# jackra1n/raytracer-rust

Hardware: NVIDIA B200
Metric: Mpaths/s (semesterbild 800x600x256spp, depth 30) (higher is better)
Workload: dtype f32

## Files before the change

raytracer-rust_b200/csrc/pt_bvh8.h:

```cpp
#pragma once
#include "pt_math.h"
#include "pt_types.h"

namespace pt {

struct MeshHit {
  float t;
  uint32_t tri;
  uint32_t order;
};

PT_HD float box_rcp(float x) {
#if defined(__CUDA_ARCH__)
  float r;
  asm("rcp.approx.ftz.f32 %0, %1;" : "=f"(r) : "f"(x));
  return r;
#else
  return 1.0f / x;
#endif
}

template <int J>
PT_HD float byte_as_unit_float(uint32_t packed) {
#if defined(__CUDA_ARCH__)
// ... 22 lines not shown
  uint32_t octinv;
  uint2 ng;
  uint2 tg;
  uint2 tg2;
};

PT_HD void trav_begin(TravState &s, V3 o, V3 d, float t_min, float t_max) {
  s.o = o;
  s.d = d;
  s.idx = box_rcp(d.x), s.idy = box_rcp(d.y), s.idz = box_rcp(d.z);
  s.t_min = t_min;
  s.best_t = t_max;
  s.best_order = 0u;
  s.best_tri = 0xffffffffu;
  const uint32_t sx = f2u(d.x) >> 31, sy = f2u(d.y) >> 31, sz = f2u(d.z) >> 31;
  s.octinv = 7u - (sx | (sy << 1) | (sz << 2));
  s.ng = make_uint2(0u, 0x80000000u);
  s.tg = make_uint2(0u, 0u);
  s.tg2 = make_uint2(0u, 0u);
}
PT_HD bool trav_has_node(const TravState &s) { return s.ng.y > 0x00FFFFFFu; }
PT_HD bool trav_has_tri(const TravState &s) { return s.tg.y != 0u; }

template <bool COUNT>
PT_HD void trav_node(const DMesh &m, TravState &s, uint2 *stack, int &sp, TraversalCounters *ctr) {
  const uint32_t hits = s.ng.y, imask = hits & 0xffu;
  const int bit = 31 - clz32(hits);
  s.ng.y &= ~(1u << bit);
  if (s.ng.y > 0x00FFFFFFu) stack[sp++] = s.ng;
  const uint32_t slot = (uint32_t)(bit - 24) ^ s.octinv;
  const uint32_t rel = (uint32_t)popc32(imask & ~(0xFFFFFFFFu << slot));
  const float4 *np = m.nodes + (size_t)(s.ng.x + rel) * 5;
  const float4 q0 = ldg4(np), q1 = ldg4(np + 1), q2 = ldg4(np + 2), q3 = ldg4(np + 3), q4 = ldg4(np + 4);
  if (COUNT) ctr->nodes++;

  const uint32_t e = f2u(q0.w);
  const float adjx = u2f(((e & 0xffu) + 15u) << 23) * s.idx;
  const float adjy = u2f((((e >> 8) & 0xffu) + 15u) << 23) * s.idy;
  const float adjz = u2f((((e >> 16) & 0xffu) + 15u) << 23) * s.idz;
  const float orgx = (q0.x - s.o.x) * s.idx - adjx, orgy = (q0.y - s.o.y) * s.idy - adjy, orgz = (q0.z - s.o.z) * s.idz - adjz;

  const bool sx = (f2u(s.d.x) >> 31) != 0u, sy = (f2u(s.d.y) >> 31) != 0u, sz = (f2u(s.d.z) >> 31) != 0u;
  const uint32_t lox0 = f2u(q2.x), lox1 = f2u(q2.y), loy0 = f2u(q2.z), loy1 = f2u(q2.w);
  const uint32_t loz0 = f2u(q3.x), loz1 = f2u(q3.y), hix0 = f2u(q3.z), hix1 = f2u(q3.w);
  const uint32_t hiy0 = f2u(q4.x), hiy1 = f2u(q4.y), hiz0 = f2u(q4.z), hiz1 = f2u(q4.w);
  const uint32_t nx[2] = {sx ? hix0 : lox0, sx ? hix1 : lox1}, fx[2] = {sx ? lox0 : hix0, sx ? lox1 : hix1};
  const uint32_t ny[2] = {sy ? hiy0 : loy0, sy ? hiy1 : loy1}, fy[2] = {sy ? loy0 : hiy0, sy ? loy1 : hiy1};
  const uint32_t nz[2] = {sz ? hiz0 : loz0, sz ? hiz1 : loz1}, fz[2] = {sz ? loz0 : hiz0, sz ? loz1 : hiz1};
  const uint32_t meta[2] = {f2u(q1.z), f2u(q1.w)};
  const uint32_t octinv4 = s.octinv * 0x01010101u;

  uint32_t hitmask = 0u;
#pragma unroll
  for (int h = 0; h < 2; h++) {
    const uint32_t meta4 = meta[h];
    const uint32_t is_inner4 = (meta4 & (meta4 << 1)) & 0x10101010u;
    const uint32_t inner_mask4 = (is_inner4 >> 4) * 0xffu;
    const uint32_t bit_index4 = (meta4 ^ (octinv4 & inner_mask4)) & 0x1f1f1f1fu;
    const uint32_t child_bits4 = (meta4 >> 5) & 0x07070707u;
#define PT_CHILD2(J)                                                                                                  \
  {                                                                                                                   \
    float tnx0, tnx1, tny0, tny1, tnz0, tnz1, tfx0, tfx1, tfy0, tfy1, tfz0, tfz1;                                     \
    fma2_bcast(tnx0, tnx1, byte_as_unit_float<J>(nx[h]), byte_as_unit_float<J + 1>(nx[h]), adjx, orgx);               \
    fma2_bcast(tny0, tny1, byte_as_unit_float<J>(ny[h]), byte_as_unit_float<J + 1>(ny[h]), adjy, orgy);               \
    fma2_bcast(tnz0, tnz1, byte_as_unit_float<J>(nz[h]), byte_as_unit_float<J + 1>(nz[h]), adjz, orgz);               \
    fma2_bcast(tfx0, tfx1, byte_as_unit_float<J>(fx[h]), byte_as_unit_float<J + 1>(fx[h]), adjx, orgx);               \
    fma2_bcast(tfy0, tfy1, byte_as_unit_float<J>(fy[h]), byte_as_unit_float<J + 1>(fy[h]), adjy, orgy);               \
    fma2_bcast(tfz0, tfz1, byte_as_unit_float<J>(fz[h]), byte_as_unit_float<J + 1>(fz[h]), adjz, orgz);               \
             \
    const float tn0 = fmaxf(fmaxf(tnx0, tny0), fmaxf(tnz0, s.t_min)), tf0 = fminf(fminf(tfx0, tfy0), fminf(tfz0, s.best_t)); \
    const float tn1 = fmaxf(fmaxf(tnx1, tny1), fmaxf(tnz1, s.t_min)), tf1 = fminf(fminf(tfx1, tfy1), fminf(tfz1, s.best_t)); \
    if (tn0 <= tf0) hitmask |= ((child_bits4 >> (8 * (J))) & 0xffu) << ((bit_index4 >> (8 * (J))) & 0xffu);           \
    if (tn1 <= tf1) hitmask |= ((child_bits4 >> (8 * (J + 1))) & 0xffu) << ((bit_index4 >> (8 * (J + 1))) & 0xffu);   \
  }
    PT_CHILD2(0) PT_CHILD2(2)
#undef PT_CHILD
  }
  s.ng.x = f2u(q1.x);
  s.ng.y = (hitmask & 0xFF000000u) | (e >> 24);
  const uint2 leaf_hits = make_uint2(f2u(q1.y), hitmask & 0x00FFFFFFu);
  if (s.tg.y == 0u) s.tg = leaf_hits;
  else s.tg2 = leaf_hits;
}

template <bool COUNT>
PT_HD void trav_tri(const DMesh &m, TravState &s, TraversalCounters *ctr) {
  const int bit = 31 - clz32(s.tg.y);
  const float4 *tp = m.tris + (size_t)(s.tg.x + (uint32_t)bit) * 3;
  s.tg.y &= ~(1u << bit);
  if (s.tg.y == 0u) {
    s.tg = s.tg2;
    s.tg2 = make_uint2(0u, 0u);
  }
  const float4 t0 = ldg4(tp), t1 = ldg4(tp + 1), t2 = ldg4(tp + 2);
  if (COUNT) ctr->tris++;
  const V3 v0 = v3(t0.x, t0.y, t0.z), edge1 = v3(t1.x, t1.y, t1.z), edge2 = v3(t2.x, t2.y, t2.z);
  const V3 h = cross(s.d, edge2);
  const float a = dot(edge1, h);
  if (fabsf(a) < kEps) return;
  const float f = 1.0f / a;
  const V3 sv = s.o - v0;
  const float u = f * dot(sv, h);
  if (!(0.0f <= u && u <= 1.0f)) return;
  const V3 q = cross(sv, edge1);
  const float v = f * dot(s.d, q);
  if (v < 0.0f || u + v > 1.0f) return;
  const float t = f * dot(edge2, q);
  if (!(t > s.t_min)) return;
  const uint32_t order = f2u(t1.w);
  if (t < s.best_t || (t == s.best_t && order < s.best_order)) {
    s.best_t = t;
    s.best_order = order;
    s.best_tri = f2u(t0.w);
  }
}

template <bool COUNT>
PT_HD bool bvh8_closest(const DMesh &m, V3 o, V3 d, float t_min, float t_max, MeshHit &out, TraversalCounters *ctr) {
  TravState s;
  trav_begin(s, o, d, t_min, t_max);
  uint2 stack[kTraversalStack];
  int sp = 0;
  for (;;) {
    if (trav_has_tri(s)) {
      trav_tri<COUNT>(m, s, ctr);
    } else if (trav_has_node(s)) {
      trav_node<COUNT>(m, s, stack, sp, ctr);
    } else {
      if (sp == 0) break;
      s.ng = stack[--sp];
    }
  }
  if (s.best_tri == 0xffffffffu) return false;
  out.t = s.best_t;
  out.tri = s.best_tri;
  out.order = s.best_order;
  return true;
}

}
```

raytracer-rust_b200/csrc/pt_scene_host.h:

```cpp
#pragma once
#include <algorithm>
#include <cmath>
#include <cstring>
#include <memory>
#include <stdexcept>
#include <vector>

#include "../../include/ptcore.h"
#include "pt_build.h"
#include "pt_types.h"

namespace pt {

inline DMesh make_dmesh(const MeshBuild &m, const float4 *nodes, const float4 *tris, const float4 *normals) {
  DMesh d;
  d.nodes = nodes;
  d.tris = tris;
  d.normals = normals;
  d.n_nodes = (int32_t)m.nodes.size();
  d.n_tris = (int32_t)m.tri48.size();
  for (int a = 0; a < 3; a++) d.root_lo[a] = m.root_lo[a], d.root_hi[a] = m.root_hi[a];
  return d;
}

struct HostScene {
  std::vector<DMaterial> materials;
  std::vector<DObject> objects;
  std::vector<std::unique_ptr<MeshBuild>> meshes;
  std::vector<float> sky;
  int32_t sky_w = 0, sky_h = 0;
  std::vector<DLight> lights;
  std::vector<float> sky_dist;

  int add_material(const ptc_material *m) {
    if (m->type < PTC_MAT_LAMBERT || m->type > PTC_MAT_NULL) throw std::invalid_argument("unknown material type");
    DMaterial d;
    memset(&d, 0, sizeof(d));
    d.type = m->type;
    d.distribution = m->distribution;
    d.fuzz = m->fuzz;
    d.ior = m->ior;
    d.roughness = m->roughness;
    d.inv_scale = m->inv_scale;
    for (int i = 0; i < 3; i++) {
// ... 146 lines not shown
```

raytracer-rust_b200/csrc/pt_types.h:

```cpp
#pragma once
#include "pt_hd.h"

namespace pt {

enum ObjType : int32_t { OBJ_SPHERE = 0, OBJ_PLANE = 1, OBJ_QUAD = 2, OBJ_CUBE = 3, OBJ_MESH = 4 };

struct alignas(16) DObject {
  int32_t type;
  int32_t material;
  int32_t mesh;
  int32_t hit_bits;
  float f[32];
};
static_assert(sizeof(DObject) == 144, "DObject layout");

struct alignas(16) DMaterial {
  int32_t type;
  int32_t distribution;
  float fuzz, ior;
  float albedo[3];
  float roughness;
  float off_color[3];
  float inv_scale;
  float eta[3];
  float pad0;
  float k[3];
  float pad1;
};
static_assert(sizeof(DMaterial) == 80, "DMaterial layout");

struct alignas(16) Node8 {
  float4 q[5];
};
static_assert(sizeof(Node8) == 80, "Node8 layout");

struct alignas(16) Tri48 {
  float4 t[3];
};

struct DMesh {
  const float4 *nodes;
  const float4 *tris;
  const float4 *normals;
  int32_t n_nodes, n_tris;
  float root_lo[3], root_hi[3];
};

struct alignas(16) DLight {
  int32_t type;
  int32_t object;
  float area;
  float pad;
  float f[12];
  float emission[3];
  float pad2;
};
constexpr int kMaxLights = 63;

struct SkyDist {
  const float *marg, *cos, *inv_sa, *cond;
  int32_t wc, hc;
};
PT_HD int32_t sky_cells(int32_t texels) { return texels > 1 ? texels - 1 : 1; }
PT_HD size_t sky_dist_size(int32_t w, int32_t h) {
  const size_t wc = (size_t)sky_cells(w), hc = (size_t)sky_cells(h);
  return 3 * hc + 2 + hc * (wc + 1);
}
PT_HD SkyDist sky_dist_view(const float *p, int32_t w, int32_t h) {
// ... 40 lines not shown
```

raytracer-rust_b200/csrc/pt_wavefront.cuh:

```cuda
#pragma once
#include <cuda_runtime.h>

#include "../../include/ptcore.h"
#include "pt_bsdf.h"
#include "pt_philox.h"
#include "pt_prims.h"

namespace ptw {
using namespace pt;

constexpr int kBlock = 256;
constexpr int kSegPerSM = 4;
constexpr uint32_t kRefillLanes = 8;
constexpr uint32_t kNoSteal = 0x80000000u;
constexpr unsigned long long kNoTriHit = ~0ull;

struct Ctl {
  unsigned long long next_path;
  unsigned long long total_paths;
  unsigned long long rays;
  unsigned long long nodes, tris, mesh_rays;
  uint32_t n_active;
  uint32_t sync_timeouts;
  uint32_t iterations[2];
// ... 101 lines not shown
      if (!mesh_root_may_hit(sc.meshes[ob->mesh], mr, t_min, closest)) continue;
      park_ray = mr;
      return k;
    }
    if (type == OBJ_SPHERE) hit = hit_sphere(ob->f, ray, t_min, closest, best);
    else if (type == OBJ_QUAD) hit = hit_quad(ob->f, ray, t_min, closest, best);
    else if (type == OBJ_CUBE) hit = hit_cube_t(ob->f, ray, t_min, closest, best);
    else hit = hit_plane(ob->f, ray, t_min, closest, best);
    if (hit) {
      improved = true;
      closest = best.t;
      best.object = k;
      best.triangle = -1;
      best.material = ob->hit_bits;
    }
  }
  return -1;
}

__device__ __forceinline__ void finish_hit(const DObject *objs, const Ray &ray, Hit &best) {
  if (best.front_face == kCubeNormalPending) cube_finish_normal(objs[best.object].f, ray, best);
}

constexpr int kSmemObjects = 24;
template <bool kSharedObjs>
__device__ __forceinline__ const DObject *stage_objects(const DScene &sc, DObject *s_objs) {
  if (!kSharedObjs) return sc.objects;
  const uint4 *src = reinterpret_cast<const uint4 *>(sc.objects);
  uint4 *dst = reinterpret_cast<uint4 *>(s_objs);
  const int n16 = sc.n_objects * (int)(sizeof(DObject) / 16);
  for (int i = threadIdx.x; i < n16; i += blockDim.x) dst[i] = src[i];
  return s_objs;
}

__device__ __forceinline__ void park_tasks(uint32_t *s_ntask, const TaskQ &tq, int par, uint32_t seg_base, int park, uint32_t i,
                                           const MeshRay &mr, float closest) {
  const uint32_t lane = threadIdx.x & 31u;
  const uint32_t mask = __ballot_sync(0xffffffffu, park >= 0);
  if (mask == 0u) return;
  uint32_t slot0 = 0;
  if (lane == 0) slot0 = atomicAdd(s_ntask, (uint32_t)__popc(mask));
  slot0 = __shfl_sync(0xffffffffu, slot0, 0);
  if (park >= 0) {
    const uint32_t slot = seg_base + slot0 + (uint32_t)__popc(mask & ((1u << lane) - 1u));
    tq.ray[par][slot] = make_uint2(i, (uint32_t)park);
    tq.o[par][slot] = make_float4(mr.o.x, mr.o.y, mr.o.z, closest);
    tq.d[par][slot] = make_float4(mr.d.x, mr.d.y, mr.d.z, 0.0f);
    tq.res[par][slot] = kNoTriHit;
  }
}

template <bool kSharedObjs>
__device__ __forceinline__ void stage_pre(uint32_t seg, uint32_t n_seg, const DScene &sc, const ExtendOut &out, const TaskQ &tq,
                                          float t_min, float t_max) {
  __shared__ uint32_t s_ntask;
  __shared__ __align__(16) DObject s_objs[kSmemObjects];
  const uint32_t tid = threadIdx.x;
  const uint32_t n = out.b.cnt[seg], seg_base = seg * out.b.cap;
  if (tid == 0) s_ntask = 0;
  const DObject *objs = kSharedObjs ? s_objs : sc.objects;
  stage_objects<kSharedObjs>(sc, s_objs);
  __syncthreads();
  for (uint32_t c0 = 0; c0 < n; c0 += (uint32_t)kBlock) {
    const uint32_t i = seg_base + c0 + tid;
    int park = -1;
    MeshRay mr;
    float closest = t_max;
    if (c0 + tid < n) {
      const float4 o4 = out.b.ray_o[i], d4 = out.b.ray_d[i];
      const Ray ray{v3(o4.x, o4.y, o4.z), v3(d4.x, d4.y, d4.z)};
      Hit best;
      bool improved = false;
      park = scan_objects(sc, objs, ray, t_min, closest, best, improved, 0, mr);
      if (improved) finish_hit(objs, ray, best);
      if (improved) write_hit(out, i, best);
      else write_miss(out, i);
    }
    park_tasks(&s_ntask, tq, 0, seg_base, park, i, mr, closest);
  }
  __syncthreads();
  if (tid == 0 && tq.cnt) tq.cnt[seg] = s_ntask;
  (void)n_seg;
}

template <bool COUNT>
__device__ __forceinline__ void stage_traverse(uint32_t seg, uint32_t n_seg, Ctl *ctl, const DScene &sc, const TaskQ &tq, int round,
                                               float t_min, uint32_t cap, uint32_t refill_arg, uint32_t part = 0u, uint32_t parts = 1u) {
  __shared__ uint32_t s_cur;
  const uint32_t n_all = tq.cnt[(uint32_t)round * n_seg + seg];
  const uint32_t first = (uint32_t)((unsigned long long)n_all * part / parts);
  const uint32_t n = (uint32_t)((unsigned long long)n_all * (part + 1u) / parts) - first, seg_base = seg * cap + first;
  const int par = round & 1;
  const uint32_t lane = threadIdx.x & 31u;
  const uint32_t lt_mask = (1u << lane) - 1u;
  const uint32_t refill_lanes = refill_arg & ~kNoSteal;
  const bool steal = (refill_arg & kNoSteal) == 0u;
  const uint32_t quota = (n >= (uint32_t)kBlock || !steal) ? 32u : max(1u, (n + (uint32_t)(kBlock / 32) - 1u) / (uint32_t)(kBlock / 32));
  if (threadIdx.x == 0) s_cur = 0;
  __syncthreads();
  TraversalCounters tc{0u, 0u, 0u};
  TravState s;
  DMesh mesh;
  mesh.nodes = nullptr, mesh.tris = nullptr;
  uint2 stack[kTraversalStack];
  int sp = 0, sb = 0;
  bool active = false;
  uint32_t task = 0;
  bool exhausted = n == 0u;
  s.ng = make_uint2(0u, 0u);
  for (;;) {
    const uint32_t idle = __ballot_sync(0xffffffffu, !active);
    if (!exhausted && (idle == 0xffffffffu || (uint32_t)__popc(idle) >= refill_lanes)) {
      const uint32_t cnt = min((uint32_t)__popc(idle), quota);
      uint32_t base = 0;
      if (lane == 0) base = atomicAdd(&s_cur, cnt);
      base = __shfl_sync(0xffffffffu, base, 0);
      const uint32_t my_rank = (uint32_t)__popc(idle & lt_mask);
      if (!active && my_rank < cnt) {
        const uint32_t j = base + my_rank;
        if (j < n) {
          const uint32_t slot = seg_base + j;
          const uint2 rk = tq.ray[par][slot];
          const float4 o4 = tq.o[par][slot], d4 = __ldcs(&tq.d[par][slot]);
          const DMesh *gm = sc.meshes + sc.objects[rk.y].mesh;
          mesh.nodes = gm->nodes;
          mesh.tris = gm->tris;
          trav_begin(s, v3(o4.x, o4.y, o4.z), v3(d4.x, d4.y, d4.z), t_min, o4.w);
          sp = sb = 0;
          task = slot;
          active = true;
          if (COUNT) tc.mesh_rays++;
        }
      }
      if (base + cnt >= n) exhausted = true;
    } else if (steal && exhausted && idle != 0u && idle != 0xffffffffu) {
      const bool can_give = active && (sp > sb || __popc(s.ng.y >> 24) >= 2);
      const uint32_t donors = __ballot_sync(0xffffffffu, can_give);
      if (donors != 0u) {
        const uint32_t pairs = (uint32_t)min(__popc(idle), __popc(donors));
        const bool give = can_give && (uint32_t)__popc(donors & lt_mask) < pairs;
        const uint32_t my_idle_rank = (uint32_t)__popc(idle & lt_mask);
        const bool take = !active && my_idle_rank < pairs;
        uint2 entry = make_uint2(0u, 0u);
        if (give) {
          if (sp > sb) {
            entry = stack[sb++];
          } else {
            const uint32_t pend = s.ng.y & 0xFF000000u, bit = pend & (0u - pend);
            entry = make_uint2(s.ng.x, bit | (s.ng.y & 0xffu));
            s.ng.y &= ~bit;
          }
        }
        const int src = take ? (int)__fns(donors, 0u, (int)my_idle_rank + 1) : (int)lane;
        const float ox = __shfl_sync(0xffffffffu, s.o.x, src), oy = __shfl_sync(0xffffffffu, s.o.y, src), oz = __shfl_sync(0xffffffffu, s.o.z, src);
// ... 15 lines not shown
          mesh.nodes = reinterpret_cast<const float4 *>(pn);
          mesh.tris = reinterpret_cast<const float4 *>(ptri);
          task = tk;
          sp = sb = 0;
          active = true;
        }
      }
    }
    if (__ballot_sync(0xffffffffu, active) == 0u) {
      if (exhausted) break;
      continue;
    }
    if (active) {
      if (!trav_has_node(s)) {
        if (sp > sb) {
          s.ng = stack[--sp];
        } else if (!trav_has_tri(s)) {
          if (s.best_tri != 0xffffffffu) atomicMin(&tq.res[par][task], ((unsigned long long)f2u(s.best_t) << 32) | (unsigned long long)s.best_order);
          active = false;
          s.ng.y = 0u;
        }
        if (sp == sb) sp = sb = 0;
      }
      if (active && trav_has_node(s) && s.tg2.y == 0u) trav_node<COUNT>(mesh, s, stack, sp, &tc);
      if (active && trav_has_tri(s)) trav_tri<COUNT>(mesh, s, &tc);
    }
  }
  if (COUNT) {
    atomicAdd(&ctl->nodes, (unsigned long long)tc.nodes);
    atomicAdd(&ctl->tris, (unsigned long long)tc.tris);
    atomicAdd(&ctl->mesh_rays, (unsigned long long)tc.mesh_rays);
  }
}

template <bool kSharedObjs>
__device__ __forceinline__ void stage_post(uint32_t seg, uint32_t n_seg, const DScene &sc, const ExtendOut &out, const TaskQ &tq,
                                           int round, float t_min, float t_max) {
  __shared__ uint32_t s_ntask;
  __shared__ __align__(16) DObject s_objs[kSmemObjects];
  const uint32_t tid = threadIdx.x;
  const uint32_t n = tq.cnt[(uint32_t)round * n_seg + seg], seg_base = seg * out.b.cap;
  const int par = round & 1;
  if (tid == 0) s_ntask = 0;
  const DObject *objs = kSharedObjs ? s_objs : sc.objects;
  stage_objects<kSharedObjs>(sc, s_objs);
  __syncthreads();
  for (uint32_t c0 = 0; c0 < n; c0 += (uint32_t)kBlock) {
    const uint32_t j = seg_base + c0 + tid;
    int park = -1;
    MeshRay mr;
    float closest = t_max;
    uint32_t i = 0;
    if (c0 + tid < n) {
      const uint2 rk = tq.ray[par][j];
      const unsigned long long res = tq.res[par][j];
      i = rk.x;
      const int k = (int)rk.y;
      const DObject *ob = objs + k;
      const bool tri_hit = res != kNoTriHit;
      const uint32_t order = (uint32_t)res;
      const float4 o4 = out.b.ray_o[i], d4 = out.b.ray_d[i];
      closest = tq.o[par][j].w;
      float4 nq = make_float4(0.0f, 0.0f, 0.0f, 0.0f);
      if (tri_hit) nq = ldg4(sc.meshes[ob->mesh].normals + order);
      const Ray ray{v3(o4.x, o4.y, o4.z), v3(d4.x, d4.y, d4.z)};
      Hit best;
      best.triangle = -1;
      bool improved = false;
      if (tri_hit) {
        const MeshRay omr = mesh_object_ray<false>(ob->f, ray);
        MeshHit mh;
        mh.t = u2f((uint32_t)(res >> 32)), mh.tri = f2u(nq.w), mh.order = order;
        Hit tmp;
        if (mesh_finish(ob->f, nq, ray, omr, mh, t_min, closest, tmp)) {
          improved = true;
          closest = tmp.t;
          best = tmp;
          best.object = k;
          best.material = ob->hit_bits;
        }
      }
      park = scan_objects(sc, objs, ray, t_min, closest, best, improved, k + 1, mr);
      if (improved) finish_hit(objs, ray, best);
      if (improved) write_hit(out, i, best);
    }
    park_tasks(&s_ntask, tq, par ^ 1, seg_base, park, i, mr, closest);
  }
  __syncthreads();
  if (tid == 0) tq.cnt[(uint32_t)(round + 1) * n_seg + seg] = s_ntask;
}

constexpr int kShadeClasses = 11;
constexpr int kShadeWindow = 2048;
constexpr int kShadeGroups = kShadeWindow / kBlock;

__device__ __forceinline__ uint32_t block_rank(bool flag, uint32_t *s_warp , uint32_t *total) {
  const uint32_t lane = threadIdx.x & 31u, warp = threadIdx.x >> 5;
  const uint32_t mask = __ballot_sync(0xffffffffu, flag);
  if (lane == 0) s_warp[warp] = (uint32_t)__popc(mask);
  __syncthreads();
  if (threadIdx.x == 0) {
    uint32_t tot = 0;
    for (int w = 0; w < kBlock / 32; w++) {
      const uint32_t c = s_warp[w];
      s_warp[w] = tot;
      tot += c;
    }
    s_warp[kBlock / 32] = tot;
  }
  __syncthreads();
// ... 287 lines not shown
    uint32_t spins = 0;
    while (ld_relaxed_u32(sr.flags + seg) < need) {
      if (++spins == (1u << 25)) {
        atomicAdd(&ctl->sync_timeouts, 1u);
        break;
      }
      __nanosleep(64);
    }
    fence_acquire();
  }
  __syncthreads();
}
__device__ __forceinline__ void stage_begin(const SegRange &sr, uint32_t seg, Ctl *ctl) {
  asm volatile("griddepcontrol.launch_dependents;" ::: "memory");
  if (sr.flags == nullptr || sr.flag_wait == 0u) asm volatile("griddepcontrol.wait;" ::: "memory");
  else segment_wait(sr, seg, ctl);
}
__device__ __forceinline__ void stage_end(const SegRange &sr, uint32_t seg) {
  if (sr.flags == nullptr) return;
  __syncthreads();
  if (threadIdx.x == 0) st_release_u32(sr.flags + seg, sr.stage_id);
}

__global__ void __launch_bounds__(kBlock, kSegPerSM) k_extend_pre(Ctl *ctl, SegRange sr, DScene sc, ExtendOut out, TaskQ tq, float t_min,
                                                                  float t_max, volatile uint32_t *progress, uint32_t seq) {
  const uint32_t seg = sr.seg0 + blockIdx.x;
  stage_begin(sr, seg, ctl);
  if (threadIdx.x == 0) {
    const uint32_t n = out.b.cnt[seg];
    if (n) {
      atomicAdd(&ctl->rays, (unsigned long long)n);
      atomicMax(&ctl->iterations[0], seq);
    }
    if (progress && blockIdx.x == 0) {
      *progress = seq << 2 | (ctl->next_path >= ctl->total_paths ? 2u : 0u) | (ctl->n_active == 0u ? 1u : 0u);
      __threadfence_system();
    }
  }
  if (sc.n_objects <= kSmemObjects) stage_pre<true>(seg, sr.n_seg, sc, out, tq, t_min, t_max);
  else stage_pre<false>(seg, sr.n_seg, sc, out, tq, t_min, t_max);
  stage_end(sr, seg);
}
template <bool COUNT>
__global__ void __launch_bounds__(kBlock, kSegPerSM) k_traverse(Ctl *ctl, SegRange sr, DScene sc, TaskQ tq, int round, float t_min,
                                                                uint32_t cap, uint32_t refill_lanes) {
  if (sr.trav_parts <= 1u) {
    stage_begin(sr, sr.seg0 + blockIdx.x, ctl);
    stage_traverse<COUNT>(sr.seg0 + blockIdx.x, sr.n_seg, ctl, sc, tq, round, t_min, cap, refill_lanes);
    stage_end(sr, sr.seg0 + blockIdx.x);
    return;
  }
  asm volatile("griddepcontrol.launch_dependents;" ::: "memory");
  if (sr.flags == nullptr || sr.flag_wait == 0u) asm volatile("griddepcontrol.wait;" ::: "memory");
  __shared__ uint32_t s_item;
  if (threadIdx.x == 0) s_item = blockIdx.x;
  __syncthreads();
  for (;;) {
    {
      const uint32_t item = s_item;
      if (item >= sr.n_seg * sr.trav_parts) break;
      const uint32_t seg = sr.seg0 + item % sr.n_seg;
      segment_wait(sr, seg, ctl);
      stage_traverse<COUNT>(seg, sr.n_seg, ctl, sc, tq, round, t_min, cap, refill_lanes, item / sr.n_seg, sr.trav_parts);
    }
    __syncthreads();
    if (threadIdx.x == 0) {
      if (sr.flags) {
        const uint32_t seg = sr.seg0 + s_item % sr.n_seg;
        __threadfence();
        if (atomicInc(sr.flags + 2u * sr.n_seg + seg, sr.trav_parts - 1u) == sr.trav_parts - 1u) {
          __threadfence();
          st_release_u32(sr.flags + seg, sr.stage_id);
        }
      }
      s_item = gridDim.x + atomicAdd(sr.trav_counter, 1u);
    }
    __syncthreads();
  }
}
__global__ void __launch_bounds__(kBlock, kSegPerSM) k_extend_post(Ctl *ctl, SegRange sr, DScene sc, ExtendOut out, TaskQ tq, int round,
                                                                   float t_min, float t_max) {
  stage_begin(sr, sr.seg0 + blockIdx.x, ctl);
  if (sc.n_objects <= kSmemObjects) stage_post<true>(sr.seg0 + blockIdx.x, sr.n_seg, sc, out, tq, round, t_min, t_max);
  else stage_post<false>(sr.seg0 + blockIdx.x, sr.n_seg, sc, out, tq, round, t_min, t_max);
  stage_end(sr, sr.seg0 + blockIdx.x);
}
template <int Mode>
__global__ void __launch_bounds__(kBlock, kSegPerSM) k_shade(Ctl *ctl, SegRange sr, DScene sc, RenderParams rp, Buffers b, Film film) {
  stage_begin(sr, sr.seg0 + blockIdx.x, ctl);
  stage_shade<Mode>(sr.seg0 + blockIdx.x, sr.n_seg, sr.flags ? sr.flags + sr.n_seg : nullptr, ctl, sc, rp, b, film);
  stage_end(sr, sr.seg0 + blockIdx.x);
}

__global__ void k_film_to_accum(Film film, size_t n_pixels, float *accum) {
  const size_t i = (size_t)blockIdx.x * blockDim.x + threadIdx.x;
  if (i >= n_pixels * 3) return;
  const size_t px = i / 3;
  accum[i] += film_value(film.sum[i], film.flags[px], (int)(i - px * 3));
}
__global__ void k_scale(const float *in, float *out, size_t n, float scale) {
  const size_t i = (size_t)blockIdx.x * blockDim.x + threadIdx.x;
  if (i < n) out[i] = in[i] * scale;
}
__global__ void k_resolve(const float *rgb, size_t n_pixels, float scale, uint32_t *out) {
  const size_t i = (size_t)blockIdx.x * blockDim.x + threadIdx.x;
  if (i < n_pixels) out[i] = resolve_pixel(rgb[i * 3] * scale, rgb[i * 3 + 1] * scale, rgb[i * 3 + 2] * scale);
}
// ... 89 lines not shown
```

raytracer-rust_b200/csrc/ptcore.cu:

```cuda
#include <cuda_runtime.h>
#include <dlfcn.h>
#include <nccl.h>

#include <algorithm>
#include <chrono>
#include <memory>
#include <mutex>
#include <thread>
#include <cstdio>
#include <cstdlib>
#include <cstring>
#include <deque>
#include <functional>
#include <string>
#include <vector>

#include "../../include/ptcore.h"
#include "pt_build_dev.h"
#include "pt_scene_host.h"
#include "pt_wavefront.cuh"

using namespace pt;
using namespace ptw;

// ... 156 lines not shown

enum Stage { ST_PRE = 0, ST_TRAVERSE, ST_POST, ST_SHADE, ST_COUNT };

template <typename... KArgs, typename... Args>
void launch_stage(bool pdl, cudaStream_t stream, uint32_t segments, void (*kernel)(KArgs...), Args &&...args) {
  cudaLaunchAttribute attr;
  attr.id = cudaLaunchAttributeProgrammaticStreamSerialization;
  attr.val.programmaticStreamSerializationAllowed = 1;
  cudaLaunchConfig_t cfg;
  memset(&cfg, 0, sizeof(cfg));
  cfg.gridDim = dim3(segments), cfg.blockDim = dim3(kBlock), cfg.dynamicSmemBytes = 0, cfg.stream = stream;
  cfg.attrs = pdl ? &attr : nullptr, cfg.numAttrs = pdl ? 1 : 0;
  CK(cudaLaunchKernelEx(&cfg, kernel, std::forward<Args>(args)...));
}

uint32_t traverse_refill_arg() {
  const char *r = getenv("PTC_REFILL"), *st = getenv("PTC_STEAL");
  return (r ? (uint32_t)atoi(r) : kRefillLanes) | ((st && atoi(st) == 0) ? kNoSteal : 0u);
}

int launch_extend(cudaStream_t stream, uint32_t segments, int rounds, Ctl *ctl, const DScene &ds, const ExtendOut &eo, const TaskQ &tq,
                  float t_min, float t_max, bool counters) {
  const SegRange sr{0u, segments, 0u, 0u, 1u};
  k_extend_pre<<<segments, kBlock, 0, stream>>>(ctl, sr, ds, eo, tq, t_min, t_max, nullptr, 0u);
  for (int r = 0; r < rounds; r++) {
    const SegRange tsr{0u, segments, 0u, (uint32_t)r, 1u};
    if (counters) k_traverse<true><<<segments, kBlock, 0, stream>>>(ctl, tsr, ds, tq, r, t_min, eo.b.cap, traverse_refill_arg());
    else k_traverse<false><<<segments, kBlock, 0, stream>>>(ctl, tsr, ds, tq, r, t_min, eo.b.cap, traverse_refill_arg());
    k_extend_post<<<segments, kBlock, 0, stream>>>(ctl, sr, ds, eo, tq, r, t_min, t_max);
  }
  return 1 + 2 * rounds;
}

void require_committed(const ptc_scene *s) {
  if (!s) throw std::invalid_argument("null scene");
  if (!s->committed) throw std::logic_error("scene not committed (call ptc_scene_commit first)");
}

void check_render_flags(const ptc_render_settings *st) {
  if ((st->flags & PTC_FLAG_NEE_SKY) && !(st->flags & PTC_FLAG_NEE)) throw std::invalid_argument("PTC_FLAG_NEE_SKY needs PTC_FLAG_NEE");
}

void ensure_ctl(ptc_scene *s) {
  if (s->h_ctl) return;
  s->d_ctl.alloc(1);
  CK(cudaMallocHost(&s->h_ctl, sizeof(Ctl) * ptc_scene::kRing));
  CK(cudaHostAlloc(&s->h_progress, 64, cudaHostAllocMapped | cudaHostAllocPortable));
  for (auto &e : s->ring_ev) CK(cudaEventCreateWithFlags(&e, cudaEventDisableTiming));
  CK(cudaEventCreate(&s->ev_begin));
  CK(cudaEventCreate(&s->ev_end));
}

// ... 129 lines not shown
    auto seg_range = [&](uint32_t trav_seq_, uint32_t trav_parts_) {
      SegRange r{0u, segments, 0u, trav_seq_, trav_parts_, s->ws.seg_flags.p, ++stage_id, (dataflow && stage_id > 1u) ? 1u : 0u, nullptr};
      if (trav_parts_ > 1u) r.trav_counter = s->ws.trav_counters.p + trav_seq_;
      return r;
    };
    int64_t mesh_tris = 0;
    for (const auto &mb : s->hs.meshes) mesh_tris += mb->n;
    const char *tp_env = getenv("PTC_TRAV_PARTS");
    const uint32_t trav_parts_bulk = tp_env ? (uint32_t)std::max(1, atoi(tp_env)) : (mesh_tris >= kHeavyMeshTriangles ? (uint32_t)kTravParts : 1u);
    if (trav_parts_bulk > 1u) CK(cudaMemsetAsync(s->ws.trav_counters.p, 0, kTravCounters * sizeof(uint32_t), stream));
    uint32_t trav_seq = 0;
    bool draining = false;
    int flip = 0;
    const bool progress_on = getenv("PTC_PROGRESS") ? atoi(getenv("PTC_PROGRESS")) != 0 : true;
    uint32_t *d_progress = nullptr;
    if (progress_on) {
      CK(cudaHostGetDevicePointer((void **)&d_progress, s->h_progress, 0));
      *(volatile uint32_t *)s->h_progress = 0u;
    }
    uint64_t it = 0;
    auto run_extend = [&]() {
      const ExtendOut eo{bufs[flip], nullptr};
      if (timing) mark(ST_PRE);
      launch_stage(pdl, stream, segments, k_extend_pre, s->d_ctl.p, seg_range(0u, 1u), s->ds, eo, tq, kEps, INFINITY,
                   (volatile uint32_t *)d_progress, (uint32_t)(it + 1));
      for (int r = 0; r < rounds; r++) {
        if (timing) mark(ST_TRAVERSE);
        const SegRange tsr = seg_range(trav_seq, (draining || trav_seq >= kTravCounters) ? 1u : trav_parts_bulk);
        trav_seq++;
        if (counters) launch_stage(pdl, stream, segments, k_traverse<true>, s->d_ctl.p, tsr, s->ds, tq, r, kEps, eo.b.cap, refill);
        else launch_stage(pdl, stream, segments, k_traverse<false>, s->d_ctl.p, tsr, s->ds, tq, r, kEps, eo.b.cap, refill);
        if (timing) mark(ST_POST);
        launch_stage(pdl, stream, segments, k_extend_post, s->d_ctl.p, seg_range(0u, 1u), s->ds, eo, tq, r, kEps, INFINITY);
      }
      launches += 1 + 2 * (uint64_t)rounds;
    };
    auto run_shade = [&]() {
      if (timing) mark(ST_SHADE);
      const SegRange ssr = seg_range(0u, 1u);
      if (nee_sky) launch_stage(pdl, stream, segments, k_shade<2>, s->d_ctl.p, ssr, s->ds, rp, bufs[flip], film);
      else if (nee) launch_stage(pdl, stream, segments, k_shade<1>, s->d_ctl.p, ssr, s->ds, rp, bufs[flip], film);
      else launch_stage(pdl, stream, segments, k_shade<0>, s->d_ctl.p, ssr, s->ds, rp, bufs[flip], film);
      launches += 1;
      flip ^= 1;
    };
    run_shade();
    bool finished = false;
    uint64_t last_iteration = ~0ull;
    if (progress_on) {
      const volatile uint32_t *prog = s->h_progress;
      while (!finished) {
        run_extend();
        run_shade();
        it++;
        const uint64_t kAhead = getenv("PTC_AHEAD") ? (uint64_t)std::max(1, atoi(getenv("PTC_AHEAD"))) : 3u;
        for (uint32_t spins = 0;; spins++) {
// ... 821 lines not shown
```

Before: 3163.

## Test BVH8 root node during object scan before parking mesh tasks

Each mesh's root node is precomputed into a decoded DRoot (float planes, bases, meta) stored in DMesh and staged into shared memory alongside the objects. The extend pre and post stages test the ray against this root and park a traversal task only when some root child is hit. The root hitmask is passed in the task's d.w so traversal starts below the root, skipping one node fetch per task. This avoids queueing and refill work for rays that miss every mesh child box, at the cost of more shared memory (24 DRoots), more ALU in the scan stages, and a larger DMesh kernel parameter.

```diff
diff --git a/raytracer-rust_b200/csrc/pt_bvh8.h b/raytracer-rust_b200/csrc/pt_bvh8.h
--- a/raytracer-rust_b200/csrc/pt_bvh8.h
+++ b/raytracer-rust_b200/csrc/pt_bvh8.h
@@ -68,34 +68,10 @@
 PT_HD bool trav_has_node(const TravState &s) { return s.ng.y > 0x00FFFFFFu; }
 PT_HD bool trav_has_tri(const TravState &s) { return s.tg.y != 0u; }
 
-template <bool COUNT>
-PT_HD void trav_node(const DMesh &m, TravState &s, uint2 *stack, int &sp, TraversalCounters *ctr) {
-  const uint32_t hits = s.ng.y, imask = hits & 0xffu;
-  const int bit = 31 - clz32(hits);
-  s.ng.y &= ~(1u << bit);
-  if (s.ng.y > 0x00FFFFFFu) stack[sp++] = s.ng;
-  const uint32_t slot = (uint32_t)(bit - 24) ^ s.octinv;
-  const uint32_t rel = (uint32_t)popc32(imask & ~(0xFFFFFFFFu << slot));
-  const float4 *np = m.nodes + (size_t)(s.ng.x + rel) * 5;
-  const float4 q0 = ldg4(np), q1 = ldg4(np + 1), q2 = ldg4(np + 2), q3 = ldg4(np + 3), q4 = ldg4(np + 4);
-  if (COUNT) ctr->nodes++;
-
-  const uint32_t e = f2u(q0.w);
-  const float adjx = u2f(((e & 0xffu) + 15u) << 23) * s.idx;
-  const float adjy = u2f((((e >> 8) & 0xffu) + 15u) << 23) * s.idy;
-  const float adjz = u2f((((e >> 16) & 0xffu) + 15u) << 23) * s.idz;
-  const float orgx = (q0.x - s.o.x) * s.idx - adjx, orgy = (q0.y - s.o.y) * s.idy - adjy, orgz = (q0.z - s.o.z) * s.idz - adjz;
-
-  const bool sx = (f2u(s.d.x) >> 31) != 0u, sy = (f2u(s.d.y) >> 31) != 0u, sz = (f2u(s.d.z) >> 31) != 0u;
-  const uint32_t lox0 = f2u(q2.x), lox1 = f2u(q2.y), loy0 = f2u(q2.z), loy1 = f2u(q2.w);
-  const uint32_t loz0 = f2u(q3.x), loz1 = f2u(q3.y), hix0 = f2u(q3.z), hix1 = f2u(q3.w);
-  const uint32_t hiy0 = f2u(q4.x), hiy1 = f2u(q4.y), hiz0 = f2u(q4.z), hiz1 = f2u(q4.w);
-  const uint32_t nx[2] = {sx ? hix0 : lox0, sx ? hix1 : lox1}, fx[2] = {sx ? lox0 : hix0, sx ? lox1 : hix1};
-  const uint32_t ny[2] = {sy ? hiy0 : loy0, sy ? hiy1 : loy1}, fy[2] = {sy ? loy0 : hiy0, sy ? loy1 : hiy1};
-  const uint32_t nz[2] = {sz ? hiz0 : loz0, sz ? hiz1 : loz1}, fz[2] = {sz ? loz0 : hiz0, sz ? loz1 : hiz1};
-  const uint32_t meta[2] = {f2u(q1.z), f2u(q1.w)};
-  const uint32_t octinv4 = s.octinv * 0x01010101u;
-
+template <class P>
+PT_HD uint32_t box8_hits(const P &p, float adjx, float adjy, float adjz, float orgx, float orgy, float orgz, float t_min, float t_max,
+                         const uint32_t meta[2], uint32_t octinv) {
+  const uint32_t octinv4 = octinv * 0x01010101u;
   uint32_t hitmask = 0u;
 #pragma unroll
   for (int h = 0; h < 2; h++) {
@@ -107,26 +83,101 @@
 #define PT_CHILD2(J)                                                                                                  \
   {                                                                                                                   \
     float tnx0, tnx1, tny0, tny1, tnz0, tnz1, tfx0, tfx1, tfy0, tfy1, tfz0, tfz1;                                     \
-    fma2_bcast(tnx0, tnx1, byte_as_unit_float<J>(nx[h]), byte_as_unit_float<J + 1>(nx[h]), adjx, orgx);               \
-    fma2_bcast(tny0, tny1, byte_as_unit_float<J>(ny[h]), byte_as_unit_float<J + 1>(ny[h]), adjy, orgy);               \
-    fma2_bcast(tnz0, tnz1, byte_as_unit_float<J>(nz[h]), byte_as_unit_float<J + 1>(nz[h]), adjz, orgz);               \
-    fma2_bcast(tfx0, tfx1, byte_as_unit_float<J>(fx[h]), byte_as_unit_float<J + 1>(fx[h]), adjx, orgx);               \
-    fma2_bcast(tfy0, tfy1, byte_as_unit_float<J>(fy[h]), byte_as_unit_float<J + 1>(fy[h]), adjy, orgy);               \
-    fma2_bcast(tfz0, tfz1, byte_as_unit_float<J>(fz[h]), byte_as_unit_float<J + 1>(fz[h]), adjz, orgz);               \
+    fma2_bcast(tnx0, tnx1, p.template plane<0, J>(0, h), p.template plane<0, J + 1>(0, h), adjx, orgx);               \
+    fma2_bcast(tny0, tny1, p.template plane<0, J>(1, h), p.template plane<0, J + 1>(1, h), adjy, orgy);               \
+    fma2_bcast(tnz0, tnz1, p.template plane<0, J>(2, h), p.template plane<0, J + 1>(2, h), adjz, orgz);               \
+    fma2_bcast(tfx0, tfx1, p.template plane<1, J>(0, h), p.template plane<1, J + 1>(0, h), adjx, orgx);               \
+    fma2_bcast(tfy0, tfy1, p.template plane<1, J>(1, h), p.template plane<1, J + 1>(1, h), adjy, orgy);               \
+    fma2_bcast(tfz0, tfz1, p.template plane<1, J>(2, h), p.template plane<1, J + 1>(2, h), adjz, orgz);               \
              \
-    const float tn0 = fmaxf(fmaxf(tnx0, tny0), fmaxf(tnz0, s.t_min)), tf0 = fminf(fminf(tfx0, tfy0), fminf(tfz0, s.best_t)); \
-    const float tn1 = fmaxf(fmaxf(tnx1, tny1), fmaxf(tnz1, s.t_min)), tf1 = fminf(fminf(tfx1, tfy1), fminf(tfz1, s.best_t)); \
+    const float tn0 = fmaxf(fmaxf(tnx0, tny0), fmaxf(tnz0, t_min)), tf0 = fminf(fminf(tfx0, tfy0), fminf(tfz0, t_max)); \
+    const float tn1 = fmaxf(fmaxf(tnx1, tny1), fmaxf(tnz1, t_min)), tf1 = fminf(fminf(tfx1, tfy1), fminf(tfz1, t_max)); \
     if (tn0 <= tf0) hitmask |= ((child_bits4 >> (8 * (J))) & 0xffu) << ((bit_index4 >> (8 * (J))) & 0xffu);           \
     if (tn1 <= tf1) hitmask |= ((child_bits4 >> (8 * (J + 1))) & 0xffu) << ((bit_index4 >> (8 * (J + 1))) & 0xffu);   \
   }
     PT_CHILD2(0) PT_CHILD2(2)
-#undef PT_CHILD
-  }
+#undef PT_CHILD2
+  }
+  return hitmask;
+}
+
+struct PackedPlanes {
+  uint32_t w[2][3][2];
+  template <int F, int J>
+  PT_HD float plane(int a, int h) const { return byte_as_unit_float<J>(w[F][a][h]); }
+};
+struct RootPlanes {
+  const DRoot *r;
+  uint32_t s[3];
+  template <int F, int J>
+  PT_HD float plane(int a, int h) const { return (s[a] ^ (uint32_t)F) ? r->plane[a][1][4 * h + J] : r->plane[a][0][4 * h + J]; }
+};
+
+template <bool COUNT>
+PT_HD void trav_node(const DMesh &m, TravState &s, uint2 *stack, int &sp, TraversalCounters *ctr) {
+  const uint32_t hits = s.ng.y, imask = hits & 0xffu;
+  const int bit = 31 - clz32(hits);
+  s.ng.y &= ~(1u << bit);
+  if (s.ng.y > 0x00FFFFFFu) stack[sp++] = s.ng;
+  const uint32_t slot = (uint32_t)(bit - 24) ^ s.octinv;
+  const uint32_t rel = (uint32_t)popc32(imask & ~(0xFFFFFFFFu << slot));
+  const float4 *np = m.nodes + (size_t)(s.ng.x + rel) * 5;
+  const float4 q0 = ldg4(np), q1 = ldg4(np + 1), q2 = ldg4(np + 2), q3 = ldg4(np + 3), q4 = ldg4(np + 4);
+  if (COUNT) ctr->nodes++;
+
+  const uint32_t e = f2u(q0.w);
+  const float adjx = u2f(((e & 0xffu) + 15u) << 23) * s.idx;
+  const float adjy = u2f((((e >> 8) & 0xffu) + 15u) << 23) * s.idy;
+  const float adjz = u2f((((e >> 16) & 0xffu) + 15u) << 23) * s.idz;
+  const float orgx = (q0.x - s.o.x) * s.idx - adjx, orgy = (q0.y - s.o.y) * s.idy - adjy, orgz = (q0.z - s.o.z) * s.idz - adjz;
+
+  const bool sx = (f2u(s.d.x) >> 31) != 0u, sy = (f2u(s.d.y) >> 31) != 0u, sz = (f2u(s.d.z) >> 31) != 0u;
+  const uint32_t lox0 = f2u(q2.x), lox1 = f2u(q2.y), loy0 = f2u(q2.z), loy1 = f2u(q2.w);
+  const uint32_t loz0 = f2u(q3.x), loz1 = f2u(q3.y), hix0 = f2u(q3.z), hix1 = f2u(q3.w);
+  const uint32_t hiy0 = f2u(q4.x), hiy1 = f2u(q4.y), hiz0 = f2u(q4.z), hiz1 = f2u(q4.w);
+  const PackedPlanes pp{{{{sx ? hix0 : lox0, sx ? hix1 : lox1}, {sy ? hiy0 : loy0, sy ? hiy1 : loy1}, {sz ? hiz0 : loz0, sz ? hiz1 : loz1}},
+                         {{sx ? lox0 : hix0, sx ? lox1 : hix1}, {sy ? loy0 : hiy0, sy ? loy1 : hiy1}, {sz ? loz0 : hiz0, sz ? loz1 : hiz1}}}};
+  const uint32_t meta[2] = {f2u(q1.z), f2u(q1.w)};
+  const uint32_t hitmask = box8_hits(pp, adjx, adjy, adjz, orgx, orgy, orgz, s.t_min, s.best_t, meta, s.octinv);
   s.ng.x = f2u(q1.x);
   s.ng.y = (hitmask & 0xFF000000u) | (e >> 24);
   const uint2 leaf_hits = make_uint2(f2u(q1.y), hitmask & 0x00FFFFFFu);
   if (s.tg.y == 0u) s.tg = leaf_hits;
   else s.tg2 = leaf_hits;
+}
+
+inline DRoot make_droot(const Node8 &n) {
+  DRoot r;
+  memset(&r, 0, sizeof(r));
+  const uint32_t e = f2u(n.q[0].w);
+  const float org[3] = {n.q[0].x, n.q[0].y, n.q[0].z};
+  for (int a = 0; a < 3; a++) r.org[a] = org[a], r.scale[a] = u2f((((e >> (8 * a)) & 0xffu) + 15u) << 23);
+  r.meta[0] = f2u(n.q[1].z), r.meta[1] = f2u(n.q[1].w);
+  r.child_base = f2u(n.q[1].x), r.tri_base = f2u(n.q[1].y), r.imask = e >> 24;
+  const float w[12] = {n.q[2].x, n.q[2].y, n.q[2].z, n.q[2].w, n.q[3].x, n.q[3].y, n.q[3].z, n.q[3].w, n.q[4].x, n.q[4].y, n.q[4].z, n.q[4].w};
+  for (int side = 0; side < 2; side++)
+    for (int a = 0; a < 3; a++)
+      for (int j = 0; j < 8; j++) {
+        const uint32_t word = f2u(w[side * 6 + a * 2 + (j >> 2)]);
+        r.plane[a][side][j] = u2f(0x3F800000u | (((word >> (8 * (j & 3))) & 0xffu) << 8));
+      }
+  return r;
+}
+
+PT_HD uint32_t trav_root(const DRoot &r, V3 o, V3 d, float t_min, float t_max) {
+  const float idx = box_rcp(d.x), idy = box_rcp(d.y), idz = box_rcp(d.z);
+  const float adjx = r.scale[0] * idx, adjy = r.scale[1] * idy, adjz = r.scale[2] * idz;
+  const float orgx = (r.org[0] - o.x) * idx - adjx, orgy = (r.org[1] - o.y) * idy - adjy, orgz = (r.org[2] - o.z) * idz - adjz;
+  const uint32_t sx = f2u(d.x) >> 31, sy = f2u(d.y) >> 31, sz = f2u(d.z) >> 31;
+  const RootPlanes rp{&r, {sx, sy, sz}};
+  const uint32_t meta[2] = {r.meta[0], r.meta[1]};
+  return box8_hits(rp, adjx, adjy, adjz, orgx, orgy, orgz, t_min, t_max, meta, 7u - (sx | (sy << 1) | (sz << 2)));
+}
+
+PT_HD void trav_begin_below_root(TravState &s, V3 o, V3 d, float t_min, float t_max, const DRoot &r, uint32_t hitmask) {
+  trav_begin(s, o, d, t_min, t_max);
+  s.ng = make_uint2(r.child_base, (hitmask & 0xFF000000u) | r.imask);
+  s.tg = make_uint2(r.tri_base, hitmask & 0x00FFFFFFu);
 }
 
 template <bool COUNT>
@@ -162,9 +213,7 @@
 }
 
 template <bool COUNT>
-PT_HD bool bvh8_closest(const DMesh &m, V3 o, V3 d, float t_min, float t_max, MeshHit &out, TraversalCounters *ctr) {
-  TravState s;
-  trav_begin(s, o, d, t_min, t_max);
+PT_HD void trav_walk(const DMesh &m, TravState &s, TraversalCounters *ctr) {
   uint2 stack[kTraversalStack];
   int sp = 0;
   for (;;) {
@@ -177,6 +226,13 @@
       s.ng = stack[--sp];
     }
   }
+}
+
+template <bool COUNT>
+PT_HD bool bvh8_closest(const DMesh &m, V3 o, V3 d, float t_min, float t_max, MeshHit &out, TraversalCounters *ctr) {
+  TravState s;
+  trav_begin(s, o, d, t_min, t_max);
+  trav_walk<COUNT>(m, s, ctr);
   if (s.best_tri == 0xffffffffu) return false;
   out.t = s.best_t;
   out.tri = s.best_tri;
diff --git a/raytracer-rust_b200/csrc/pt_scene_host.h b/raytracer-rust_b200/csrc/pt_scene_host.h
--- a/raytracer-rust_b200/csrc/pt_scene_host.h
+++ b/raytracer-rust_b200/csrc/pt_scene_host.h
@@ -8,6 +8,7 @@
 
 #include "../../include/ptcore.h"
 #include "pt_build.h"
+#include "pt_bvh8.h"
 #include "pt_types.h"
 
 namespace pt {
@@ -20,6 +21,7 @@
   d.n_nodes = (int32_t)m.nodes.size();
   d.n_tris = (int32_t)m.tri48.size();
   for (int a = 0; a < 3; a++) d.root_lo[a] = m.root_lo[a], d.root_hi[a] = m.root_hi[a];
+  d.root = make_droot(m.nodes[0]);
   return d;
 }
 
diff --git a/raytracer-rust_b200/csrc/pt_types.h b/raytracer-rust_b200/csrc/pt_types.h
--- a/raytracer-rust_b200/csrc/pt_types.h
+++ b/raytracer-rust_b200/csrc/pt_types.h
@@ -38,12 +38,23 @@
   float4 t[3];
 };
 
+struct alignas(16) DRoot {
+  float org[3];
+  float scale[3];
+  uint32_t meta[2];
+  uint32_t child_base, tri_base, imask;
+  uint32_t pad;
+  float plane[3][2][8];
+};
+static_assert(sizeof(DRoot) == 240, "DRoot layout");
+
 struct DMesh {
   const float4 *nodes;
   const float4 *tris;
   const float4 *normals;
   int32_t n_nodes, n_tris;
   float root_lo[3], root_hi[3];
+  DRoot root;
 };
 
 struct alignas(16) DLight {
diff --git a/raytracer-rust_b200/csrc/pt_wavefront.cuh b/raytracer-rust_b200/csrc/pt_wavefront.cuh
--- a/raytracer-rust_b200/csrc/pt_wavefront.cuh
+++ b/raytracer-rust_b200/csrc/pt_wavefront.cuh
@@ -147,19 +147,45 @@
   if (best.front_face == kCubeNormalPending) cube_finish_normal(objs[best.object].f, ray, best);
 }
 
+template <bool COUNT>
+__device__ __forceinline__ int scan_to_task(const DScene &sc, const DObject *objs, const DRoot *roots, const Ray &ray, float t_min,
+                                            float &closest, Hit &best, bool &improved, int k, MeshRay &mr, uint32_t &hitmask,
+                                            uint32_t &n_root) {
+  for (;;) {
+    const int park = scan_objects(sc, objs, ray, t_min, closest, best, improved, k, mr);
+    if (park < 0) return -1;
+    const int mi = objs[park].mesh;
+    hitmask = trav_root(roots ? roots[mi] : sc.meshes[mi].root, mr.o, mr.d, t_min, closest);
+    if (COUNT) n_root++;
+    if (hitmask != 0u) return park;
+    k = park + 1;
+  }
+}
+
+__device__ __forceinline__ void count_root_steps(Ctl *ctl, uint32_t n_root) {
+  const uint32_t sum = __reduce_add_sync(0xffffffffu, n_root);
+  if ((threadIdx.x & 31u) == 0u && sum != 0u) {
+    atomicAdd(&ctl->nodes, (unsigned long long)sum);
+    atomicAdd(&ctl->mesh_rays, (unsigned long long)sum);
+  }
+}
+
 constexpr int kSmemObjects = 24;
 template <bool kSharedObjs>
-__device__ __forceinline__ const DObject *stage_objects(const DScene &sc, DObject *s_objs) {
-  if (!kSharedObjs) return sc.objects;
+__device__ __forceinline__ void stage_objects(const DScene &sc, DObject *s_objs, DRoot *s_roots) {
+  if (!kSharedObjs) return;
   const uint4 *src = reinterpret_cast<const uint4 *>(sc.objects);
   uint4 *dst = reinterpret_cast<uint4 *>(s_objs);
   const int n16 = sc.n_objects * (int)(sizeof(DObject) / 16);
   for (int i = threadIdx.x; i < n16; i += blockDim.x) dst[i] = src[i];
-  return s_objs;
+  constexpr int kRoot16 = (int)(sizeof(DRoot) / 16);
+  uint4 *rdst = reinterpret_cast<uint4 *>(s_roots);
+  for (int i = threadIdx.x; i < sc.n_meshes * kRoot16; i += blockDim.x)
+    rdst[i] = reinterpret_cast<const uint4 *>(&sc.meshes[i / kRoot16].root)[i % kRoot16];
 }
 
 __device__ __forceinline__ void park_tasks(uint32_t *s_ntask, const TaskQ &tq, int par, uint32_t seg_base, int park, uint32_t i,
-                                           const MeshRay &mr, float closest) {
+                                           const MeshRay &mr, float closest, uint32_t hitmask) {
   const uint32_t lane = threadIdx.x & 31u;
   const uint32_t mask = __ballot_sync(0xffffffffu, park >= 0);
   if (mask == 0u) return;
@@ -170,39 +196,44 @@
     const uint32_t slot = seg_base + slot0 + (uint32_t)__popc(mask & ((1u << lane) - 1u));
     tq.ray[par][slot] = make_uint2(i, (uint32_t)park);
     tq.o[par][slot] = make_float4(mr.o.x, mr.o.y, mr.o.z, closest);
-    tq.d[par][slot] = make_float4(mr.d.x, mr.d.y, mr.d.z, 0.0f);
+    tq.d[par][slot] = make_float4(mr.d.x, mr.d.y, mr.d.z, u2f(hitmask));
     tq.res[par][slot] = kNoTriHit;
   }
 }
 
-template <bool kSharedObjs>
-__device__ __forceinline__ void stage_pre(uint32_t seg, uint32_t n_seg, const DScene &sc, const ExtendOut &out, const TaskQ &tq,
+template <bool kSharedObjs, bool COUNT>
+__device__ __forceinline__ void stage_pre(uint32_t seg, uint32_t n_seg, Ctl *ctl, const DScene &sc, const ExtendOut &out, const TaskQ &tq,
                                           float t_min, float t_max) {
   __shared__ uint32_t s_ntask;
   __shared__ __align__(16) DObject s_objs[kSmemObjects];
+  __shared__ __align__(16) DRoot s_roots[kSharedObjs ? kSmemObjects : 1];
   const uint32_t tid = threadIdx.x;
   const uint32_t n = out.b.cnt[seg], seg_base = seg * out.b.cap;
   if (tid == 0) s_ntask = 0;
   const DObject *objs = kSharedObjs ? s_objs : sc.objects;
-  stage_objects<kSharedObjs>(sc, s_objs);
-  __syncthreads();
+  const DRoot *roots = kSharedObjs ? s_roots : nullptr;
+  stage_objects<kSharedObjs>(sc, s_objs, s_roots);
+  __syncthreads();
+  uint32_t n_root = 0;
   for (uint32_t c0 = 0; c0 < n; c0 += (uint32_t)kBlock) {
     const uint32_t i = seg_base + c0 + tid;
     int park = -1;
     MeshRay mr;
     float closest = t_max;
+    uint32_t hitmask = 0u;
     if (c0 + tid < n) {
       const float4 o4 = out.b.ray_o[i], d4 = out.b.ray_d[i];
       const Ray ray{v3(o4.x, o4.y, o4.z), v3(d4.x, d4.y, d4.z)};
       Hit best;
       bool improved = false;
-      park = scan_objects(sc, objs, ray, t_min, closest, best, improved, 0, mr);
+      park = scan_to_task<COUNT>(sc, objs, roots, ray, t_min, closest, best, improved, 0, mr, hitmask, n_root);
       if (improved) finish_hit(objs, ray, best);
       if (improved) write_hit(out, i, best);
       else write_miss(out, i);
     }
-    park_tasks(&s_ntask, tq, 0, seg_base, park, i, mr, closest);
-  }
+    park_tasks(&s_ntask, tq, 0, seg_base, park, i, mr, closest, hitmask);
+  }
+  if (COUNT) count_root_steps(ctl, n_root);
   __syncthreads();
   if (tid == 0 && tq.cnt) tq.cnt[seg] = s_ntask;
   (void)n_seg;
@@ -234,6 +265,7 @@
   bool exhausted = n == 0u;
   s.ng = make_uint2(0u, 0u);
   for (;;) {
+    bool fresh = false;
     const uint32_t idle = __ballot_sync(0xffffffffu, !active);
     if (!exhausted && (idle == 0xffffffffu || (uint32_t)__popc(idle) >= refill_lanes)) {
       const uint32_t cnt = min((uint32_t)__popc(idle), quota);
@@ -250,11 +282,11 @@
           const DMesh *gm = sc.meshes + sc.objects[rk.y].mesh;
           mesh.nodes = gm->nodes;
           mesh.tris = gm->tris;
-          trav_begin(s, v3(o4.x, o4.y, o4.z), v3(d4.x, d4.y, d4.z), t_min, o4.w);
+          trav_begin_below_root(s, v3(o4.x, o4.y, o4.z), v3(d4.x, d4.y, d4.z), t_min, o4.w, gm->root, f2u(d4.w));
+          fresh = trav_has_tri(s);
           sp = sb = 0;
           task = slot;
           active = true;
-          if (COUNT) tc.mesh_rays++;
         }
       }
       if (base + cnt >= n) exhausted = true;
@@ -316,35 +348,37 @@
         }
         if (sp == sb) sp = sb = 0;
       }
-      if (active && trav_has_node(s) && s.tg2.y == 0u) trav_node<COUNT>(mesh, s, stack, sp, &tc);
+      if (active && !fresh && trav_has_node(s) && s.tg2.y == 0u) trav_node<COUNT>(mesh, s, stack, sp, &tc);
       if (active && trav_has_tri(s)) trav_tri<COUNT>(mesh, s, &tc);
     }
   }
   if (COUNT) {
     atomicAdd(&ctl->nodes, (unsigned long long)tc.nodes);
     atomicAdd(&ctl->tris, (unsigned long long)tc.tris);
-    atomicAdd(&ctl->mesh_rays, (unsigned long long)tc.mesh_rays);
-  }
-}
-
-template <bool kSharedObjs>
-__device__ __forceinline__ void stage_post(uint32_t seg, uint32_t n_seg, const DScene &sc, const ExtendOut &out, const TaskQ &tq,
+  }
+}
+
+template <bool kSharedObjs, bool COUNT>
+__device__ __forceinline__ void stage_post(uint32_t seg, uint32_t n_seg, Ctl *ctl, const DScene &sc, const ExtendOut &out, const TaskQ &tq,
                                            int round, float t_min, float t_max) {
   __shared__ uint32_t s_ntask;
   __shared__ __align__(16) DObject s_objs[kSmemObjects];
+  __shared__ __align__(16) DRoot s_roots[kSharedObjs ? kSmemObjects : 1];
   const uint32_t tid = threadIdx.x;
   const uint32_t n = tq.cnt[(uint32_t)round * n_seg + seg], seg_base = seg * out.b.cap;
   const int par = round & 1;
   if (tid == 0) s_ntask = 0;
   const DObject *objs = kSharedObjs ? s_objs : sc.objects;
-  stage_objects<kSharedObjs>(sc, s_objs);
-  __syncthreads();
+  const DRoot *roots = kSharedObjs ? s_roots : nullptr;
+  stage_objects<kSharedObjs>(sc, s_objs, s_roots);
+  __syncthreads();
+  uint32_t n_root = 0;
   for (uint32_t c0 = 0; c0 < n; c0 += (uint32_t)kBlock) {
     const uint32_t j = seg_base + c0 + tid;
     int park = -1;
     MeshRay mr;
     float closest = t_max;
-    uint32_t i = 0;
+    uint32_t i = 0, hitmask = 0u;
     if (c0 + tid < n) {
       const uint2 rk = tq.ray[par][j];
       const unsigned long long res = tq.res[par][j];
@@ -374,12 +408,13 @@
           best.material = ob->hit_bits;
         }
       }
-      park = scan_objects(sc, objs, ray, t_min, closest, best, improved, k + 1, mr);
+      park = scan_to_task<COUNT>(sc, objs, roots, ray, t_min, closest, best, improved, k + 1, mr, hitmask, n_root);
       if (improved) finish_hit(objs, ray, best);
       if (improved) write_hit(out, i, best);
     }
-    park_tasks(&s_ntask, tq, par ^ 1, seg_base, park, i, mr, closest);
-  }
+    park_tasks(&s_ntask, tq, par ^ 1, seg_base, park, i, mr, closest, hitmask);
+  }
+  if (COUNT) count_root_steps(ctl, n_root);
   __syncthreads();
   if (tid == 0) tq.cnt[(uint32_t)(round + 1) * n_seg + seg] = s_ntask;
 }
@@ -713,6 +748,7 @@
   if (threadIdx.x == 0) st_release_u32(sr.flags + seg, sr.stage_id);
 }
 
+template <bool COUNT>
 __global__ void __launch_bounds__(kBlock, kSegPerSM) k_extend_pre(Ctl *ctl, SegRange sr, DScene sc, ExtendOut out, TaskQ tq, float t_min,
                                                                   float t_max, volatile uint32_t *progress, uint32_t seq) {
   const uint32_t seg = sr.seg0 + blockIdx.x;
@@ -728,8 +764,8 @@
       __threadfence_system();
     }
   }
-  if (sc.n_objects <= kSmemObjects) stage_pre<true>(seg, sr.n_seg, sc, out, tq, t_min, t_max);
-  else stage_pre<false>(seg, sr.n_seg, sc, out, tq, t_min, t_max);
+  if (sc.n_objects <= kSmemObjects) stage_pre<true, COUNT>(seg, sr.n_seg, ctl, sc, out, tq, t_min, t_max);
+  else stage_pre<false, COUNT>(seg, sr.n_seg, ctl, sc, out, tq, t_min, t_max);
   stage_end(sr, seg);
 }
 template <bool COUNT>
@@ -769,11 +805,12 @@
     __syncthreads();
   }
 }
+template <bool COUNT>
 __global__ void __launch_bounds__(kBlock, kSegPerSM) k_extend_post(Ctl *ctl, SegRange sr, DScene sc, ExtendOut out, TaskQ tq, int round,
                                                                    float t_min, float t_max) {
   stage_begin(sr, sr.seg0 + blockIdx.x, ctl);
-  if (sc.n_objects <= kSmemObjects) stage_post<true>(sr.seg0 + blockIdx.x, sr.n_seg, sc, out, tq, round, t_min, t_max);
-  else stage_post<false>(sr.seg0 + blockIdx.x, sr.n_seg, sc, out, tq, round, t_min, t_max);
+  if (sc.n_objects <= kSmemObjects) stage_post<true, COUNT>(sr.seg0 + blockIdx.x, sr.n_seg, ctl, sc, out, tq, round, t_min, t_max);
+  else stage_post<false, COUNT>(sr.seg0 + blockIdx.x, sr.n_seg, ctl, sc, out, tq, round, t_min, t_max);
   stage_end(sr, sr.seg0 + blockIdx.x);
 }
 template <int Mode>
diff --git a/raytracer-rust_b200/csrc/ptcore.cu b/raytracer-rust_b200/csrc/ptcore.cu
--- a/raytracer-rust_b200/csrc/ptcore.cu
+++ b/raytracer-rust_b200/csrc/ptcore.cu
@@ -202,12 +202,11 @@
 int launch_extend(cudaStream_t stream, uint32_t segments, int rounds, Ctl *ctl, const DScene &ds, const ExtendOut &eo, const TaskQ &tq,
                   float t_min, float t_max, bool counters) {
   const SegRange sr{0u, segments, 0u, 0u, 1u};
-  k_extend_pre<<<segments, kBlock, 0, stream>>>(ctl, sr, ds, eo, tq, t_min, t_max, nullptr, 0u);
+  (counters ? k_extend_pre<true> : k_extend_pre<false>)<<<segments, kBlock, 0, stream>>>(ctl, sr, ds, eo, tq, t_min, t_max, nullptr, 0u);
   for (int r = 0; r < rounds; r++) {
     const SegRange tsr{0u, segments, 0u, (uint32_t)r, 1u};
-    if (counters) k_traverse<true><<<segments, kBlock, 0, stream>>>(ctl, tsr, ds, tq, r, t_min, eo.b.cap, traverse_refill_arg());
-    else k_traverse<false><<<segments, kBlock, 0, stream>>>(ctl, tsr, ds, tq, r, t_min, eo.b.cap, traverse_refill_arg());
-    k_extend_post<<<segments, kBlock, 0, stream>>>(ctl, sr, ds, eo, tq, r, t_min, t_max);
+    (counters ? k_traverse<true> : k_traverse<false>)<<<segments, kBlock, 0, stream>>>(ctl, tsr, ds, tq, r, t_min, eo.b.cap, traverse_refill_arg());
+    (counters ? k_extend_post<true> : k_extend_post<false>)<<<segments, kBlock, 0, stream>>>(ctl, sr, ds, eo, tq, r, t_min, t_max);
   }
   return 1 + 2 * rounds;
 }
@@ -383,16 +382,16 @@
     auto run_extend = [&]() {
       const ExtendOut eo{bufs[flip], nullptr};
       if (timing) mark(ST_PRE);
-      launch_stage(pdl, stream, segments, k_extend_pre, s->d_ctl.p, seg_range(0u, 1u), s->ds, eo, tq, kEps, INFINITY,
+      launch_stage(pdl, stream, segments, counters ? k_extend_pre<true> : k_extend_pre<false>, s->d_ctl.p, seg_range(0u, 1u), s->ds, eo, tq, kEps, INFINITY,
                    (volatile uint32_t *)d_progress, (uint32_t)(it + 1));
       for (int r = 0; r < rounds; r++) {
         if (timing) mark(ST_TRAVERSE);
         const SegRange tsr = seg_range(trav_seq, (draining || trav_seq >= kTravCounters) ? 1u : trav_parts_bulk);
         trav_seq++;
-        if (counters) launch_stage(pdl, stream, segments, k_traverse<true>, s->d_ctl.p, tsr, s->ds, tq, r, kEps, eo.b.cap, refill);
-        else launch_stage(pdl, stream, segments, k_traverse<false>, s->d_ctl.p, tsr, s->ds, tq, r, kEps, eo.b.cap, refill);
+        launch_stage(pdl, stream, segments, counters ? k_traverse<true> : k_traverse<false>, s->d_ctl.p, tsr, s->ds, tq, r, kEps, eo.b.cap, refill);
         if (timing) mark(ST_POST);
-        launch_stage(pdl, stream, segments, k_extend_post, s->d_ctl.p, seg_range(0u, 1u), s->ds, eo, tq, r, kEps, INFINITY);
+        launch_stage(pdl, stream, segments, counters ? k_extend_post<true> : k_extend_post<false>, s->d_ctl.p, seg_range(0u, 1u), s->ds, eo, tq, r,
+                     kEps, INFINITY);
       }
       launches += 1 + 2 * (uint64_t)rounds;
     };
```

Result: faster. 3195, median of 6 (+1.0%).
